# ArielleRosinski/pyGAT

Hardware: AMD Instinct MI355X
Metric: GAT-layer fwd+bwd edges/sec (higher is better)
Workload: dtype f32

## Files before the change

include/pygat_amd.h:

```cpp
#ifndef PYGAT_AMD_H
#define PYGAT_AMD_H

#include <stdint.h>
#include <stddef.h>

#ifdef __cplusplus
extern "C" {
#endif

#define PYGAT_ABI_VERSION 15

enum {
  PYGAT_OK = 0,
  PYGAT_EINVAL = -1,
  PYGAT_EHIP = -2,
  PYGAT_ENODEV = -3
};

enum {
  PYGAT_F_ELU = 1,
  PYGAT_F_SKIP = 2,
  PYGAT_F_MAIN_ONLY = 4,
  PYGAT_F_FIXUP_ONLY = 8
};

// ... 63 lines not shown
typedef struct {
  int n;
  int64_t nnz;
  const int32_t* rowptr;
  const int32_t* edge_rc;
  int slot_edges;
  const int32_t* slot_begin;
  const int32_t* cut_rows;
  int n_cut;
  int n_cut_wide;
  int64_t slot_first;
  int64_t slot_count;
  const int32_t* slot_meta;
  const int32_t* slot_order;
  const int32_t* user_row;
} pygat_graph;

int pygat_edge_pairs(int n, const int32_t* rowptr, const int32_t* col, int32_t* edge_rc, void* stream);

int pygat_slot_bounds(int n, int64_t nnz, const int32_t* rowptr, const int32_t* edge_rc, int slot_edges,
                      int32_t* slot_begin, void* stream);
int pygat_slot_meta(int n, int64_t nnz, const int32_t* rowptr, const int32_t* edge_rc, int slot_edges,
                    const int32_t* slot_begin, int32_t* slot_meta, void* stream);

size_t pygat_partials_bytes(int64_t nnz, int slot_edges, int H, int Fp);

int pygat_head_group(int n, int H, int Fo);

int pygat_gat_forward_phases_ok(int n, int H, int Fo);
int pygat_gat_forward(const pygat_graph* g, int H, int Fo, float alpha, int flags,
                      const float* Wh, const float* s, const float* a_pad, const float* sk,
// ... 119 lines not shown
```

pygat_amd/_lib.py:

```python
from __future__ import annotations

import ctypes as C
import os

import torch

_HERE = os.path.dirname(os.path.abspath(__file__))
LIB_PATH = os.path.join(_HERE, "libpygat_amd.so")
from .config import config as _config
if _config.lib_path:
    LIB_PATH = os.path.abspath(_config.lib_path)

ABI_VERSION = 15
F_ELU = 1
F_SKIP = 2
F_MAIN_ONLY = 4
F_FIXUP_ONLY = 8

SYMBOLS = [
    "pygat_abi_version", "pygat_last_error", "pygat_padded_width", "pygat_device_count",
    "pygat_device_name", "pygat_kernel_footprint", "pygat_default_gemm_mode", "pygat_dense_row_counts", "pygat_scan_workspace_bytes",
    "pygat_exclusive_scan_i32", "pygat_dense_fill_cols", "pygat_csr_symmetric_perm",
    "pygat_gemm_workspace_bytes", "pygat_gemm_f32", "pygat_gemm_f32_blocked", "pygat_project_blocked", "pygat_wgrad_blocked", "pygat_pack_params", "pygat_pack_params_heads", "pygat_stack_heads", "pygat_stack_heads_padded", "pygat_project", "pygat_attn_scores",
    "pygat_unpack_wgrad",
    "pygat_edge_pairs", "pygat_slot_bounds", "pygat_slot_meta", "pygat_partials_bytes", "pygat_head_group", "pygat_gat_forward", "pygat_gat_forward_phases_ok", "pygat_gat_forward_tail", "pygat_gat_backward_col_tail", "pygat_gat_backward_tail", "pygat_project_tail_blocked", "pygat_head_mean",
    "pygat_gat_backward_prepare", "pygat_gat_backward_row", "pygat_gat_backward_col", "pygat_gat_backward_rowsum",
    "pygat_gat_backward_col_da_bytes", "pygat_a_grad_fold",
    "pygat_agrad_workspace_bytes", "pygat_a_grad", "pygat_wgrad_workspace_bytes", "pygat_wgrad",
# ... 13 lines not shown


class OutSegments(C.Structure):
    _fields_ = [("nseg", C.c_int), ("col_start", C.c_int32 * (MAX_SEGMENTS + 1)), ("ptr", C.c_void_p * MAX_SEGMENTS),
                ("ld", C.c_int64 * MAX_SEGMENTS)]


class ColBlocks(C.Structure):
    _fields_ = [("w", C.c_int), ("stride", C.c_int64)]


class Graph(C.Structure):
    _fields_ = [("n", C.c_int), ("nnz", C.c_int64), ("rowptr", C.c_void_p), ("edge_rc", C.c_void_p),
                ("slot_edges", C.c_int), ("slot_begin", C.c_void_p), ("cut_rows", C.c_void_p),
                ("n_cut", C.c_int), ("n_cut_wide", C.c_int), ("slot_first", C.c_int64), ("slot_count", C.c_int64),
                ("slot_meta", C.c_void_p), ("slot_order", C.c_void_p), ("user_row", C.c_void_p)]


def _load():
    if not os.path.exists(LIB_PATH):
        raise ImportError(
            f"pygat_amd: {LIB_PATH} not found. Build it with `python -c 'import __graft_entry__ as g; "
            f"g.build()'` or `make -C pygat_amd/csrc`. There is no CPU/PyTorch fallback for the hot path.")
    lib = C.CDLL(LIB_PATH)
    missing = [s for s in SYMBOLS if not hasattr(lib, s)]
    if missing:
        raise ImportError(f"pygat_amd: {LIB_PATH} lacks symbols {missing}")
    p, i, i64, f, sz = C.c_void_p, C.c_int, C.c_int64, C.c_float, C.c_size_t
    lib.pygat_abi_version.restype = i
    lib.pygat_last_error.restype = C.c_char_p
    lib.pygat_padded_width.argtypes = [i]
# ... 113 lines not shown
```

pygat_amd/config.py:

```python
from __future__ import annotations

import os
from dataclasses import dataclass, fields
from typing import Optional


def _flag(name: str, default: bool) -> bool:
    v = os.environ.get(name)
    return default if v is None else v not in ("0", "", "false", "False")


def _opt_flag(name: str) -> Optional[bool]:
    v = os.environ.get(name)
    return None if v is None else v == "1"


def _opt_int(name: str) -> Optional[int]:
    v = os.environ.get(name)
    return int(v) if v else None


@dataclass(frozen=True)
class Config:
    lib_path: Optional[str]
    dist_chunks: int
    dropout_wide: bool
    sparse_max_density: float
    sparse_x: bool
    slot_edges: Optional[int]
    slot_meta: bool
    two_gather_backward: Optional[bool]
    backward: Optional[str]
    da_in_k4: bool
    k1_split_min_k: int
    overlap_backward: bool
    pad_k: bool
    renumber: bool
    tail: bool
    tail_fused: bool

    @staticmethod
    def from_env() -> "Config":
        return Config(
            lib_path=os.environ.get("PYGAT_AMD_LIB") or None,
            dist_chunks=int(os.environ.get("PYGAT_DIST_CHUNKS", 4)),
            dropout_wide=_flag("PYGAT_DROPOUT_WIDE", False),
            sparse_max_density=float(os.environ.get("PYGAT_SPARSE_MAX_DENSITY", 0.15)),
            sparse_x=_flag("PYGAT_SPARSE_X", True),
            slot_edges=_opt_int("PYGAT_SLOT_EDGES"),
            slot_meta=not _flag("PYGAT_NO_SLOT_META", False),
            two_gather_backward=_opt_flag("PYGAT_TWO_GATHER_BACKWARD"),
            backward=os.environ.get("PYGAT_BACKWARD") or None,
            da_in_k4=_flag("PYGAT_DA_IN_K4", True),
            k1_split_min_k=int(os.environ.get("PYGAT_K1_SPLIT_MIN_K", 128)),
            overlap_backward=_flag("PYGAT_OVERLAP_BACKWARD", False),
            pad_k=_flag("PYGAT_PAD_K", True),
            renumber=_flag("PYGAT_RENUMBER", True),
            tail=_flag("PYGAT_TAIL", True),
            tail_fused=_flag("PYGAT_TAIL_FUSED", True),
        )

    def describe(self) -> dict:
        return {f.name: getattr(self, f.name) for f in fields(self)}


config = Config.from_env()
```

pygat_amd/csrc/attn_common.h:

```cpp
#pragma once
#include "common.h"

namespace pygat {

constexpr int FIX_LIST_WAVES = 16;
__host__ __device__ constexpr int fix_rows_per_wave(int lpr) { return 64 / lpr >= 8 ? 4 : (64 / lpr >= 2 ? 2 : 1); }
constexpr int FIX_WIDE = 32;
constexpr int FIX_SCREEN = 8;
constexpr float NEG_BIG = -1.0e30f;

struct RowShape {
  int H, Fo, Fp, R, NCH;
  int fp_shift;
  int lph;
  int Htot;
  int64_t ldr;
  int64_t ldh;
  int64_t ldo;
};

static inline bool make_row_shape(int H, int Fo, RowShape* rs) {
  int Fp = padded_width(Fo);
  if (H <= 0 || Fp == 0) return false;
  rs->H = H; rs->Fo = Fo; rs->Fp = Fp; rs->R = H * Fp; rs->NCH = rs->R / 4;
// ... 75 lines not shown
  } while (0)

struct GraphDev {
  int n;
  int64_t nnz;
  const int32_t* rowptr;
  const int2* rc;
  int ts;
  const int32_t* sb;
  const int4* meta;
  const int32_t* cut;
  int n_cut, n_cut_wide;
  int64_t k0, kn;
  const int32_t* order;
  const int32_t* urow;
};

static inline int check_graph(const pygat_graph* g, GraphDev* d, int allow_slot_range = 0) {
  if (!g || !g->rowptr || !g->edge_rc || g->n <= 0 || g->nnz <= 0) {
    set_error("graph: null or empty (n=%d nnz=%lld)", g ? g->n : -1, g ? (long long)g->nnz : -1LL);
    return PYGAT_EINVAL;
  }
  if (g->nnz >= (int64_t)1 << 31) {
    set_error("graph: nnz %lld exceeds int32 edge indexing", (long long)g->nnz);
    return PYGAT_EINVAL;
  }
  if (g->slot_edges < 4 || (g->slot_edges & 3)) {
    set_error("graph: slot_edges=%d must be a multiple of 4, >= 4", g->slot_edges);
    return PYGAT_EINVAL;
  }
  d->n = g->n; d->nnz = g->nnz; d->rowptr = g->rowptr; d->rc = reinterpret_cast<const int2*>(g->edge_rc);
  d->ts = g->slot_edges; d->sb = g->slot_begin; d->meta = reinterpret_cast<const int4*>(g->slot_meta);
  if (g->slot_meta && !aligned16(g->slot_meta)) {
    set_error("graph: slot_meta must be 16-byte aligned");
    return PYGAT_EINVAL;
  }
  d->cut = g->cut_rows; d->n_cut = g->cut_rows ? g->n_cut : 0; d->n_cut_wide = g->cut_rows ? g->n_cut_wide : 0;
  if (d->n_cut < 0 || d->n_cut_wide < 0 || d->n_cut_wide > d->n_cut) {
    set_error("graph: bad cut-row list (n_cut=%d n_cut_wide=%d)", g->n_cut, g->n_cut_wide);
    return PYGAT_EINVAL;
  }
  const int64_t total = (g->nnz + g->slot_edges - 1) / g->slot_edges;
  d->k0 = 0; d->kn = total;
  d->order = g->slot_order;
  d->urow = g->user_row;
  if (g->slot_order && g->slot_count != 0) {
    set_error("graph: slot_order needs the whole slot range (slot_count = 0)");
    return PYGAT_EINVAL;
  }
  if (g->slot_count != 0) {
    if (!allow_slot_range || g->slot_first < 0 || g->slot_count < 0 || g->slot_first + g->slot_count > total ||
        (allow_slot_range == 2 && g->slot_first != 0)) {
      set_error("graph: slot range [%lld, +%lld) of %lld %s", (long long)g->slot_first, (long long)g->slot_count,
                (long long)total, allow_slot_range ? "is out of bounds (or not a prefix, for the column pass)"
                                                   : "is not supported by this entry point");
      return PYGAT_EINVAL;
    }
    d->k0 = g->slot_first; d->kn = g->slot_count;
  }
  return PYGAT_OK;
// ... 78 lines not shown
template <int LPR, int SPAN = 64>
__device__ __forceinline__ float slot_sum(float x) {
#pragma unroll
  for (int off = LPR; off < SPAN; off <<= 1) x += __shfl_xor(x, off);
  return x;
}
template <int LPR, int SPAN = 64>
__device__ __forceinline__ float4 slot_sum4(float4 v) {
#pragma unroll
  for (int off = LPR; off < SPAN; off <<= 1) {
    v.x += __shfl_xor(v.x, off); v.y += __shfl_xor(v.y, off);
    v.z += __shfl_xor(v.z, off); v.w += __shfl_xor(v.w, off);
  }
  return v;
}
#endif

}
```

pygat_amd/csrc/k2_forward.hip:

```cpp
#include "attn_common.h"

namespace pygat {

struct FwdArgs {
  GraphDev g;
  RowShape rs;
  float alpha;
  int flags;
  const float* Wh;
  int64_t ldwh;
  const float* s;
  const float* a_pad;
  const float* sk;
  const float* mask;
  float* out;
  float* hattn;
  float* m;
  float* Z;
  float* part;
  float* aneg;
  float* qneg;
};

__device__ __forceinline__ float lrelu(float z, float alpha) { return z > 0.f ? z : alpha * z; }
// ... 91 lines not shown
        float* o = a.out + io * ldo + (int64_t)h * Fo + f0;
        if (f0 + 0 < Fo) o[0] = pre.x;
        if (f0 + 1 < Fo) o[1] = pre.y;
        if (f0 + 2 < Fo) o[2] = pre.z;
        if (f0 + 3 < Fo) o[3] = pre.w;
      }
    }
    if (a.m && ((co >> 2) & (a.rs.lph - 1)) == 0) {
      a.m[(int64_t)i * ldh + h] = st.m[v];
      a.Z[(int64_t)i * ldh + h] = st.z[v];
      if constexpr (AUX) a.qneg[(int64_t)i * ldh + h] = mixed[v] ? st.zn[v] * rz : 0.f;
    }
  }
}

template <int VEC, bool AUX>
__device__ __forceinline__ void part_store(const FwdArgs& a, const LaneCols<VEC>& lc, float* p, const RowState<VEC, AUX>& st) {
  const int R = a.rs.R, H = a.rs.H;
#pragma unroll
  for (int v = 0; v < VEC; ++v) {
    if (!lc.valid[v]) continue;
    st4(p + lc.cofs[v], st.acc[v]);
    if constexpr (AUX) st4(p + R + 2 * H + lc.cofs[v], st.accn[v]);
    if (((lc.cofs[v] >> 2) & (a.rs.lph - 1)) == 0) {
      p[R + lc.head[v]] = st.m[v];
      p[R + H + lc.head[v]] = st.z[v];
      if constexpr (AUX) p[2 * R + 2 * H + lc.head[v]] = st.zn[v];
    }
  }
}
template <int VEC, bool AUX>
struct PartRec {
  float m[VEC], z[VEC];
  float4 acc[VEC];
  float zn[AUX ? VEC : 1];
  float4 accn[AUX ? VEC : 1];
};
template <int VEC, bool AUX>
__device__ __forceinline__ void part_load(const FwdArgs& a, const LaneCols<VEC>& lc, const float* p, PartRec<VEC, AUX>& r) {
  const int R = a.rs.R, H = a.rs.H;
#pragma unroll
  for (int v = 0; v < VEC; ++v) {
// ... 1 lines not shown
    if constexpr (AUX) { r.zn[v] = p[2 * R + 2 * H + lc.head[v]]; r.accn[v] = ld4(p + R + 2 * H + lc.cofs[v]); }
  }
}
template <int VEC, bool AUX>
__device__ __forceinline__ void part_merge(RowState<VEC, AUX>& st, const PartRec<VEC, AUX>& r) {
#pragma unroll
  for (int v = 0; v < VEC; ++v)
    merge_state<AUX>(st.m[v], st.z[v], st.acc[v], st.zn[AUX ? v : 0], st.accn[AUX ? v : 0], r.m[v], r.z[v], r.acc[v],
                     r.zn[AUX ? v : 0], r.accn[AUX ? v : 0]);
}

template <int LPR, int VEC, bool AUX, int LPH = 0, int CR = 0>
__device__ __forceinline__ void fwd_flush(const FwdArgs& a, const LaneCols<VEC>& lc, int64_t k, int i,
                                          bool is_head, bool is_tail, const RowState<VEC, AUX>& st) {
  if (is_head || is_tail) {
    part_store<VEC, AUX>(a, lc, a.part + (2 * k + (is_head ? 0 : 1)) * part_stride<AUX>(a.rs), st);
  } else {
    fwd_finish<LPR, VEC, AUX, LPH, CR>(a, lc, i, st);
  }
}

#ifndef PYGAT_K2_PREFETCH_ALL
#define PYGAT_K2_PREFETCH_ALL 0
#endif
#ifndef PYGAT_K2_PREFETCH_TRAIN
#define PYGAT_K2_PREFETCH_TRAIN 1
#endif
#ifndef PYGAT_K2_HEADLINE_WAVES
#define PYGAT_K2_HEADLINE_WAVES 4
#endif
#ifndef PYGAT_K2_DEEP
#define PYGAT_K2_DEEP 0
#endif
#ifndef PYGAT_K2_NARROW_U
#define PYGAT_K2_NARROW_U 4
#endif
template <int LPR, int VEC, bool V2, bool AUX, bool FAST, int LPH = 0, int CR = 0>
__global__ __launch_bounds__(256) __attribute__((amdgpu_waves_per_eu((AUX && FAST && VEC == 1 && LPR > 8) ? PYGAT_K2_HEADLINE_WAVES : 1))) void gat_fwd_kernel(FwdArgs a) {
  constexpr int EPW = 64 / LPR;
  constexpr bool NARROW = (VEC == 1 && LPR <= 8);
  constexpr bool PREF = NARROW || (PYGAT_K2_PREFETCH_ALL && VEC == 1) || (PYGAT_K2_PREFETCH_TRAIN && AUX && FAST && VEC == 1);
  constexpr int U = (VEC == 1) ? (NARROW ? PYGAT_K2_NARROW_U : 4) : 2;
  const int lane = threadIdx.x & 63;
  const int64_t kl = ((int64_t)blockIdx.x * (blockDim.x >> 6) + (threadIdx.x >> 6)) * EPW + lane / LPR;
  if (kl >= a.g.kn) return;
  const int64_t k = a.g.order ? a.g.order[kl] : a.g.k0 + kl;
  int64_t e0, e1;
  const int2* __restrict__ rc = a.g.rc;
  int r_first;
  bool head_partial, tail_known = false, tail_flag = false;
  if (a.g.meta) {
    const int4 mt = a.g.meta[k];
    e0 = mt.x; e1 = mt.y; r_first = mt.z;
    head_partial = (mt.w & 1) != 0; tail_known = true; tail_flag = (mt.w & 2) != 0;
  } else {
    slot_range(a.g, k, &e0, &e1);
    r_first = rc[e0].x;
    head_partial = a.g.rowptr[r_first] < e0;
  }
  const LaneCols<VEC> lc = lane_cols<LPR, VEC>(a.rs);
  const int R = CR ? CR : a.rs.R;
// ... 117 lines not shown
          st.reset();
        }
#pragma unroll
        for (int v = 0; v < VEC; ++v) {
          const float zz = sv[u][v] + tv[u][v];
          fold_edge<AUX>(st.m[v], st.z[v], st.acc[v], st.zn[AUX ? v : 0], st.accn[AUX ? v : 0],
                         V2 ? tv[u][v] : lrelu(zz, a.alpha), !(zz > 0.f), wv[u][v], mk[u][v]);
        }
      }
    }
  }
  const bool tail_partial = tail_known ? tail_flag : a.g.rowptr[cur + 1] > e1;
  fwd_flush<LPR, VEC, AUX, LPH, CR>(a, lc, k, cur, cur == r_first && head_partial, tail_partial, st);
}

template <int LPR, int VEC, bool AUX, int NW, int G = 64 / LPR>
__device__ __forceinline__ void fwd_merge_row(const FwdArgs& a, const LaneCols<VEC>& lc, float* fix_sm, int64_t k, int r,
                                              int npieces, bool wide, int w) {
  constexpr int PF = (VEC == 1) ? 4 : 2;
  const int lane = threadIdx.x & 63, slot = lane / LPR, g = slot % G;
  const int64_t PS = part_stride<AUX>(a.rs);
  RowState<VEC, AUX> st;
  st.reset();
  if (wide || w == 0) {
    const int nw = wide ? NW : 1;
    for (int q = (wide ? w : 0) * G * PF + g; q < npieces; q += nw * G * PF) {
      PartRec<VEC, AUX> rec[PF];
#pragma unroll
      for (int f = 0; f < PF; ++f) {
        const int qq = q + f * G;
        const int qc = qq < npieces ? qq : q;
        part_load<VEC, AUX>(a, lc, a.part + (qc == 0 ? 2 * k + 1 : 2 * (k + qc)) * PS, rec[f]);
      }
#pragma unroll
      for (int f = 0; f < PF; ++f)
        if (q + f * G < npieces) part_merge<VEC, AUX>(st, rec[f]);
    }
#pragma unroll
    for (int off = LPR; off < LPR * G; off <<= 1) {
#pragma unroll
      for (int v = 0; v < VEC; ++v) {
        const float mo = __shfl_xor(st.m[v], off), zo = __shfl_xor(st.z[v], off);
        float4 ao, no = make_float4(0.f, 0.f, 0.f, 0.f);
        float zno = 0.f;
        ao.x = __shfl_xor(st.acc[v].x, off); ao.y = __shfl_xor(st.acc[v].y, off);
        ao.z = __shfl_xor(st.acc[v].z, off); ao.w = __shfl_xor(st.acc[v].w, off);
        if constexpr (AUX) {
          zno = __shfl_xor(st.zn[v], off);
          no.x = __shfl_xor(st.accn[v].x, off); no.y = __shfl_xor(st.accn[v].y, off);
          no.z = __shfl_xor(st.accn[v].z, off); no.w = __shfl_xor(st.accn[v].w, off);
        }
        merge_state<AUX>(st.m[v], st.z[v], st.acc[v], st.zn[AUX ? v : 0], st.accn[AUX ? v : 0], mo, zo, ao, zno, no);
      }
    }
  }
  if (wide) {
    if (slot == 0) part_store<VEC, AUX>(a, lc, fix_sm + w * PS, st);
    __syncthreads();
    if (w == 0 && slot == 0) {
#pragma unroll
      for (int ww = 1; ww < NW; ++ww) {
        PartRec<VEC, AUX> rec;
        part_load<VEC, AUX>(a, lc, fix_sm + ww * PS, rec);
        part_merge<VEC, AUX>(st, rec);
      }
    }
    __syncthreads();
  }
  if (w == 0 && g == 0 && npieces > 0) fwd_finish<LPR, VEC, AUX>(a, lc, r, st);
}

template <int LPR, int VEC, bool AUX>
__global__ __launch_bounds__(256) void gat_fwd_fixup_kernel(FwdArgs a) {
  constexpr int EPW = 64 / LPR;
  constexpr int PF = (VEC == 1) ? 4 : 2;
  extern __shared__ __attribute__((aligned(16))) float fix_sm[];
  const int lane = threadIdx.x & 63, w = threadIdx.x >> 6;
  const int64_t kbase = a.g.k0 + (int64_t)blockIdx.x * FIX_SCREEN;
  const int64_t nslots = a.g.k0 + a.g.kn;
  int my_r = 0, my_end = 0;
  bool owner = false;
  if (lane < FIX_SCREEN && kbase + lane < nslots) {
    int64_t e0, e1;
    slot_range(a.g, kbase + lane, &e0, &e1);
// ... 77 lines not shown
extern "C" size_t pygat_partials_bytes(int64_t nnz, int slot_edges, int H, int Fp) {
  if (nnz <= 0 || slot_edges <= 0) return 0;
  const int64_t nslots = (nnz + slot_edges - 1) / slot_edges;
  return (size_t)(2 * nslots) * (size_t)(2 * H * Fp + 3 * H) * sizeof(float);
}

static int launch_forward(const pygat_graph* g, int H, int Fo, float alpha, int flags, const float* Wh, int v2,
                          const float* s, const float* a_pad, const float* sk, const float* att_mask, float* out,
                          float* hattn, float* m, float* Z, float* aneg, float* qneg, void* part, void* stream) {
  FwdArgs a;
  int rc = check_graph(g, &a.g, v2 ? 2 : 1);
  if (rc) return rc;
  const int Fp = padded_width(Fo);
  PYGAT_REQUIRE(H > 0 && Fp > 0, "gat_forward: unsupported H=%d F'=%d", H, Fo);
  PYGAT_REQUIRE(Wh && (s || v2) && a_pad && part, "gat_forward: null Wh/s/a_pad/part");
  PYGAT_REQUIRE(out || hattn, "gat_forward: need out and/or hattn");
  PYGAT_REQUIRE(!(flags & PYGAT_F_SKIP) || sk, "gat_forward: PYGAT_F_SKIP without sk");
  PYGAT_REQUIRE((m == nullptr) == (Z == nullptr), "gat_forward: m and Z must be given together");
  PYGAT_REQUIRE((aneg == nullptr) == (qneg == nullptr) && (!aneg || (m && !v2 && aligned16(aneg))),
                "gat_forward: aneg and qneg come together, need m/Z, 16-byte alignment and the v1 layer");
  PYGAT_REQUIRE(aligned16(Wh) && aligned16(part) && aligned16(a_pad) && (!sk || aligned16(sk)) && (!hattn || aligned16(hattn)) &&
                    (!out || Fo != Fp || aligned16(out)),
                "gat_forward: row tables must be 16-byte aligned");
  hipStream_t st = (hipStream_t)stream;
  const int64_t nslots = a.g.kn;
  const int hg = v2 ? H : head_group_fwd_n(a.g.n, H, Fp);
  const bool do_main = !(flags & PYGAT_F_FIXUP_ONLY), do_fix = !(flags & PYGAT_F_MAIN_ONLY);
  PYGAT_REQUIRE(do_main || do_fix, "gat_forward: PYGAT_F_MAIN_ONLY and PYGAT_F_FIXUP_ONLY exclude each other");
  PYGAT_REQUIRE((do_main && do_fix) || hg >= H, "gat_forward: a single phase needs the level in one head window (pygat_gat_forward_phases_ok)");
  flags &= ~(PYGAT_F_MAIN_ONLY | PYGAT_F_FIXUP_ONLY);
// ... 24 lines not shown
    if (!do_main) {}
    else if (v2) PYGAT_FWD(true, false, false);
    else if (aux && fast && lpr == 32 && vec == 1 && a.rs.lph == 4)
      if (a.rs.R == 128 && a.rs.ldr == 128 && a.rs.ldh == 8 && a.rs.ldo == 128 && a.rs.Fo == 16 && a.ldwh == 128 && !(flags & PYGAT_F_SKIP))
        hipLaunchKernelGGL((gat_fwd_kernel<32, 1, false, true, true, 4, 128>), dim3(blocks), dim3(bt), 0, st, a);
      else
        hipLaunchKernelGGL((gat_fwd_kernel<32, 1, false, true, true, 4>), dim3(blocks), dim3(bt), 0, st, a);
    else if (aux && fast) PYGAT_FWD(false, true, true);
    else if (aux) PYGAT_FWD(false, true, false);
    else PYGAT_FWD(false, false, false);
#undef PYGAT_FWD
    PYGAT_CHECK_LAUNCH("gat_forward");
    const bool listed = a.g.cut != nullptr;
    const int fix_waves = listed ? FIX_LIST_WAVES : 4;
    const size_t fix_lds = fix_waves * (size_t)(aux ? part_stride<true>(a.rs) : part_stride<false>(a.rs)) * sizeof(float);
    const unsigned fb = listed ? (unsigned)(a.g.n_cut_wide + cdiv(a.g.n_cut - a.g.n_cut_wide, FIX_LIST_WAVES * fix_rows_per_wave(lpr)))
                               : (unsigned)cdiv(nslots, FIX_SCREEN);
    if ((listed && a.g.n_cut == 0) || !do_fix) continue;
#define PYGAT_FIX(AUXV)                                                                                               \
    do {                                                                                                              \
      if (listed) {                                                                                                   \
        PYGAT_DISPATCH_LANES(lpr, vec, hipLaunchKernelGGL((gat_fwd_fixup_list_kernel<LPR, VEC, AUXV>), dim3(fb),     \
                                                          dim3(64 * FIX_LIST_WAVES), fix_lds, st, a));                \
      } else {                                                                                                        \
        PYGAT_DISPATCH_LANES(lpr, vec, hipLaunchKernelGGL((gat_fwd_fixup_kernel<LPR, VEC, AUXV>), dim3(fb), dim3(256), \
                                                          fix_lds, st, a));                                           \
      }                                                                                                               \
    } while (0)
    if (aux) PYGAT_FIX(true); else PYGAT_FIX(false);
#undef PYGAT_FIX
    PYGAT_CHECK_LAUNCH("gat_forward_fixup");
  }
  return PYGAT_OK;
// ... 55 lines not shown
```

pygat_amd/graph.py:

```python
from __future__ import annotations

import ctypes as C
import weakref
from typing import Optional, Tuple

import torch

from . import _lib
from ._lib import lib, check
from .config import config as _config

SLOT_ORDER_FN = None
FORCED_SLOT_EDGES = _config.slot_edges
USE_SLOT_META = _config.slot_meta

DEFAULT_SLOT_EDGES = 64


def auto_slot_edges(nnz: int) -> int:
    if FORCED_SLOT_EDGES:
        return int(FORCED_SLOT_EDGES)
    ts = DEFAULT_SLOT_EDGES
    while ts > 4 and nnz // ts < 8192:
        ts //= 2
    return ts


def slot_edges_for(row_floats: int, base: int = DEFAULT_SLOT_EDGES) -> int:
    return min(base, 32) if row_floats <= 16 else base
# ... 7 lines not shown
    return None if t is None else t.data_ptr()


class _Pattern:

    def __init__(self, rowptr: torch.Tensor, col: torch.Tensor, slot_edges: int, user_row: Optional[torch.Tensor] = None):
        self.rowptr, self.col, self.slot_edges = rowptr, col, slot_edges
        self.user_row = user_row
        self.n = rowptr.numel() - 1
        self.nnz = col.numel()
        self.edge_rc = torch.empty(self.nnz, 2, dtype=torch.int32, device=rowptr.device)
        with torch.cuda.device(rowptr.device):
            check(lib.pygat_edge_pairs(self.n, rowptr.data_ptr(), col.data_ptr(), self.edge_rc.data_ptr(), _stream()),
                  "edge_pairs")
        self._alt = {}
        self.struct = self._make(slot_edges, True)

    def _make(self, slot_edges: int, snapped: bool):
        key = (slot_edges, snapped)
        if key not in self._alt:
            sb = None
            if snapped:
                nslots = -(-self.nnz // slot_edges)
                sb = torch.empty(nslots + 1, dtype=torch.int32, device=self.rowptr.device)
                with torch.cuda.device(self.rowptr.device):
                    check(lib.pygat_slot_bounds(self.n, self.nnz, self.rowptr.data_ptr(), self.edge_rc.data_ptr(),
                                                slot_edges, sb.data_ptr(), _stream()), "slot_bounds")
            cut, n_cut, n_wide = None, 0, 0
            if snapped:
                sbl = sb.long()
# ... 8 lines not shown
                    order = torch.argsort(pieces, descending=True, stable=True)
                    cut = torch.stack([k, r_last[k], pieces], 1)[order].to(torch.int32).contiguous()
                    n_cut, n_wide = int(k.numel()), int((pieces > 32).sum().item())
                else:
                    cut = torch.zeros(1, 3, dtype=torch.int32, device=self.rowptr.device)
            meta = torch.empty(-(-self.nnz // slot_edges), 4, dtype=torch.int32, device=self.rowptr.device)
            with torch.cuda.device(self.rowptr.device):
                check(lib.pygat_slot_meta(self.n, self.nnz, self.rowptr.data_ptr(), self.edge_rc.data_ptr(), slot_edges, _ptr(sb),
                                          meta.data_ptr(), _stream()), "slot_meta")
            if not USE_SLOT_META:
                meta = None
            order = SLOT_ORDER_FN(self, meta) if (SLOT_ORDER_FN is not None and meta is not None) else None
            st = _lib.Graph(self.n, self.nnz, _ptr(self.rowptr), _ptr(self.edge_rc), slot_edges, _ptr(sb), _ptr(cut),
                            n_cut, n_wide, 0, 0, _ptr(meta), _ptr(order), _ptr(self.user_row))
            self._alt[key] = (st, sb, cut, meta, order)
        return self._alt[key][0]

    def row_chunks(self, nchunks: int, slot_edges: Optional[int] = None, nslots: Optional[int] = None, row_end: Optional[int] = None):
        ts = slot_edges or self.slot_edges
        key = ("chunks", ts, nchunks, nslots)
        if key not in self._alt:
            base = self._make(ts, True)
            _, sb, cut, meta, _order = self._alt[(ts, True)]
            all_slots = sb.numel() - 1
            nslots = all_slots if nslots is None else int(nslots)
            sbl, rp = sb.long(), self.rowptr.long()
            first_row = self.edge_rc[sbl[:-1], 0].long()
            starts_row = rp[first_row] == sbl[:-1]
            ok = torch.nonzero(starts_row[:nslots]).flatten()
            borders = [0]
            for c in range(1, nchunks):
# ... 7 lines not shown
                r0 = int(first_row[b0])
                r1 = int(first_row[b1]) if b1 < nslots else (self.n if (row_end is None or nslots == all_slots) else int(row_end))
                sub, n_cut, n_wide = None, 0, 0
                if cut is not None:
                    sel = (cut[:, 0] >= b0) & (cut[:, 0] < b1)
                    sub = cut[sel].contiguous()
                    n_cut, n_wide = int(sub.shape[0]), int((sub[:, 2] > 32).sum().item()) if sub.numel() else 0
                    if n_cut == 0:
                        sub = cut[:1].contiguous()
                st = _lib.Graph(self.n, self.nnz, _ptr(self.rowptr), _ptr(self.edge_rc), ts, _ptr(sb), _ptr(sub), n_cut,
                                n_wide, b0, b1 - b0, _ptr(meta), None, _ptr(self.user_row))
                out.append((st, r0, r1))
                keep.append(sub)
            self._alt[key] = (out, keep)
            del base
        return [(C.byref(st), r0, r1) for st, r0, r1 in self._alt[key][0]]

    def self_loop_tail(self, slot_edges: Optional[int] = None):
        ts = slot_edges or self.slot_edges
        key = ("tail", ts)
        if key not in self._alt:
            st = self._make(ts, True)
            _, sb, cut, meta, order = self._alt[(ts, True)]
            out = None
            if meta is not None and order is None:
                rp = self.rowptr.long()
                deg = rp[1:] - rp[:-1]
                n1 = int((deg > 1).sum().item())
                if n1 < self.n and bool((deg[n1:] == 1).all().item()) and bool((self.col[rp[n1]:].long() == torch.arange(n1, self.n, device=self.col.device)).all().item()):
                    first_row = meta[:, 2].long()
                    k = int(torch.searchsorted(first_row, torch.tensor(n1, device=first_row.device)).item())
                    if 0 < k < meta.shape[0]:
                        row_first = int(first_row[k].item())
                        pre = _lib.Graph()
                        C.memmove(C.byref(pre), C.byref(st), C.sizeof(_lib.Graph))
                        pre.slot_first, pre.slot_count = 0, k
                        out = (row_first, k, pre)
            self._alt[key] = out
        t = self._alt[key]
        return None if t is None else (t[0], t[1], C.byref(t[2]))

    def ref(self, slot_edges: Optional[int] = None, snapped: bool = True):
        return C.byref(self._make(slot_edges or self.slot_edges, snapped))


class _UnmappedPattern:

    def __init__(self, base: "_Pattern"):
        self._base = base
        self._copies = {}
        self.user_row = None

    def __getattr__(self, name):
        return getattr(self._base, name)

    def _strip(self, key, struct_ref):
        if key not in self._copies:
            st = _lib.Graph()
            C.memmove(C.byref(st), struct_ref, C.sizeof(_lib.Graph))
            st.user_row = None
            self._copies[key] = st
        return C.byref(self._copies[key])

    def ref(self, slot_edges: Optional[int] = None, snapped: bool = True):
        return self._strip(("ref", slot_edges or self._base.slot_edges, snapped), self._base.ref(slot_edges, snapped))

    def row_chunks(self, nchunks: int, slot_edges: Optional[int] = None, nslots: Optional[int] = None, row_end: Optional[int] = None):
        out = self._base.row_chunks(nchunks, slot_edges, nslots, row_end)
        return [(self._strip(("chunk", slot_edges or self._base.slot_edges, nchunks, nslots, c), ref), r0, r1)
                for c, (ref, r0, r1) in enumerate(out)]

    def self_loop_tail(self, slot_edges: Optional[int] = None):
        t = self._base.self_loop_tail(slot_edges)
        return None if t is None else (t[0], t[1], self._strip(("tail", slot_edges or self._base.slot_edges), t[2]))


class InternalOrderView:
    degree_sorted = True
    user_row = None
    _ordered = None

    def __init__(self, g_int: "CSRGraph", to_user: torch.Tensor, to_internal: torch.Tensor):
        self.base = g_int
        self.n, self.nnz, self.device, self.slot_edges, self.symmetric = g_int.n, g_int.nnz, g_int.device, g_int.slot_edges, g_int.symmetric
        self.fwd = _UnmappedPattern(g_int.fwd)
        self.bwd = self.fwd if g_int.bwd is g_int.fwd else _UnmappedPattern(g_int.bwd)
        self.perm_t, self.perm_f = g_int.perm_t, g_int.perm_f
        self.to_user, self.to_internal = to_user, to_internal

# ... 173 lines not shown
```

Baseline: 4.134 billion.

## Merge cut-row partials inside the forward kernel via arrival counters

Adds per-cut-row atomic arrival counters so the last slot to finish a row split across slots merges the partial softmax states inline, inside the forward kernel. Only narrow cut rows (up to 32 pieces) are handled this way; wide rows keep the separate fix-up launch. Partial stores use agent-scope atomic write-through so other workgroups see them before merging. This is meant to remove most of the fix-up kernel launch and its extra pass over the partials, at the cost of atomics, fences and possible divergence in the main kernel.

```diff
diff --git a/include/pygat_amd.h b/include/pygat_amd.h
--- a/include/pygat_amd.h
+++ b/include/pygat_amd.h
@@ -8,7 +8,7 @@
 extern "C" {
 #endif
 
-#define PYGAT_ABI_VERSION 15
+#define PYGAT_ABI_VERSION 16
 
 enum {
   PYGAT_OK = 0,
@@ -102,7 +102,12 @@
   const int32_t* slot_meta;
   const int32_t* slot_order;
   const int32_t* user_row;
+  const int32_t* slot_cut;
+  const int32_t* cut_all;
+  uint32_t* merge_cnt;
+  int n_cut_all;
 } pygat_graph;
+enum { PYGAT_MERGE_FWD = 0, PYGAT_MERGE_FWD_V2 = 1, PYGAT_MERGE_COL = 2, PYGAT_MERGE_PASSES = 3 };
 
 int pygat_edge_pairs(int n, const int32_t* rowptr, const int32_t* col, int32_t* edge_rc, void* stream);
 
diff --git a/pygat_amd/_lib.py b/pygat_amd/_lib.py
--- a/pygat_amd/_lib.py
+++ b/pygat_amd/_lib.py
@@ -11,7 +11,7 @@
 if _config.lib_path:
     LIB_PATH = os.path.abspath(_config.lib_path)
 
-ABI_VERSION = 15
+ABI_VERSION = 16
 F_ELU = 1
 F_SKIP = 2
 F_MAIN_ONLY = 4
@@ -55,7 +55,9 @@
     _fields_ = [("n", C.c_int), ("nnz", C.c_int64), ("rowptr", C.c_void_p), ("edge_rc", C.c_void_p),
                 ("slot_edges", C.c_int), ("slot_begin", C.c_void_p), ("cut_rows", C.c_void_p),
                 ("n_cut", C.c_int), ("n_cut_wide", C.c_int), ("slot_first", C.c_int64), ("slot_count", C.c_int64),
-                ("slot_meta", C.c_void_p), ("slot_order", C.c_void_p), ("user_row", C.c_void_p)]
+                ("slot_meta", C.c_void_p), ("slot_order", C.c_void_p), ("user_row", C.c_void_p),
+                ("slot_cut", C.c_void_p), ("cut_all", C.c_void_p), ("merge_cnt", C.c_void_p), ("n_cut_all", C.c_int)]
+MERGE_PASSES = 3
 
 
 def _load():
diff --git a/pygat_amd/config.py b/pygat_amd/config.py
--- a/pygat_amd/config.py
+++ b/pygat_amd/config.py
@@ -38,6 +38,7 @@
     renumber: bool
     tail: bool
     tail_fused: bool
+    inkernel_merge: bool
 
     @staticmethod
     def from_env() -> "Config":
@@ -58,6 +59,7 @@
             renumber=_flag("PYGAT_RENUMBER", True),
             tail=_flag("PYGAT_TAIL", True),
             tail_fused=_flag("PYGAT_TAIL_FUSED", True),
+            inkernel_merge=_flag("PYGAT_INKERNEL_MERGE", True),
         )
 
     def describe(self) -> dict:
diff --git a/pygat_amd/csrc/attn_common.h b/pygat_amd/csrc/attn_common.h
--- a/pygat_amd/csrc/attn_common.h
+++ b/pygat_amd/csrc/attn_common.h
@@ -113,6 +113,10 @@
   int64_t k0, kn;
   const int32_t* order;
   const int32_t* urow;
+  const int2* slot_cut;
+  const int32_t* cut_all;
+  uint32_t* merge_cnt;
+  int n_cut_all;
 };
 
 static inline int check_graph(const pygat_graph* g, GraphDev* d, int allow_slot_range = 0) {
@@ -143,6 +147,18 @@
   d->k0 = 0; d->kn = total;
   d->order = g->slot_order;
   d->urow = g->user_row;
+  d->slot_cut = reinterpret_cast<const int2*>(g->slot_cut); d->cut_all = g->cut_all; d->merge_cnt = g->merge_cnt;
+  d->n_cut_all = g->slot_cut ? g->n_cut_all : 0;
+  if (g->slot_cut && (!g->cut_all || !g->merge_cnt || g->n_cut_all < 0 || ((uintptr_t)g->slot_cut & 7))) {
+    set_error("graph: slot_cut needs cut_all, merge_cnt, n_cut_all >= 0 and 8-byte alignment");
+    return PYGAT_EINVAL;
+  }
+  d->slot_cut = reinterpret_cast<const int2*>(g->slot_cut); d->cut_all = g->cut_all; d->merge_cnt = g->merge_cnt;
+  d->n_cut_all = g->slot_cut ? g->n_cut_all : 0;
+  if (g->slot_cut && (!g->cut_all || !g->merge_cnt || g->n_cut_all < 0 || ((uintptr_t)g->slot_cut & 7))) {
+    set_error("graph: slot_cut needs cut_all, merge_cnt, n_cut_all >= 0 and 8-byte alignment");
+    return PYGAT_EINVAL;
+  }
   if (g->slot_order && g->slot_count != 0) {
     set_error("graph: slot_order needs the whole slot range (slot_count = 0)");
     return PYGAT_EINVAL;
@@ -251,6 +267,64 @@
   }
   return v;
 }
+
+__device__ __forceinline__ void st4_wt(float* p, float4 v) {
+  unsigned long long* q = reinterpret_cast<unsigned long long*>(p);
+  __hip_atomic_store(q, (unsigned long long)__float_as_uint(v.x) | ((unsigned long long)__float_as_uint(v.y) << 32),
+                     __ATOMIC_RELAXED, __HIP_MEMORY_SCOPE_AGENT);
+  __hip_atomic_store(q + 1, (unsigned long long)__float_as_uint(v.z) | ((unsigned long long)__float_as_uint(v.w) << 32),
+                     __ATOMIC_RELAXED, __HIP_MEMORY_SCOPE_AGENT);
+}
+__device__ __forceinline__ void st1_wt(float* p, float v) { __hip_atomic_store(p, v, __ATOMIC_RELAXED, __HIP_MEMORY_SCOPE_AGENT); }
+__device__ __forceinline__ void merge_drain() { asm volatile("s_waitcnt vmcnt(0)" ::: "memory"); }
+__device__ __forceinline__ bool merge_arrive(const GraphDev& g, int pass, int c) {
+  uint32_t* cnt = g.merge_cnt + (int64_t)pass * g.n_cut_all + c;
+  const uint32_t pieces = (uint32_t)g.cut_all[3 * c + 2];
+  const uint32_t old = __hip_atomic_fetch_add(cnt, 1u, __ATOMIC_RELAXED, __HIP_MEMORY_SCOPE_AGENT);
+  if (old + 1u != pieces) return false;
+  __hip_atomic_store(cnt, 0u, __ATOMIC_RELAXED, __HIP_MEMORY_SCOPE_AGENT);
+  return true;
+}
+__device__ __forceinline__ void merge_acquire() {
+  __builtin_amdgcn_fence(__ATOMIC_ACQUIRE, "agent");
+  asm volatile("s_waitcnt vmcnt(0)" ::: "memory");
+}
+struct MergeJobs {
+  unsigned long long mh, mt;
+  int jh, jt;
+};
+template <int LPR>
+__device__ __forceinline__ bool merge_arrivals(const GraphDev& g, int pass, int2 sc, MergeJobs& j) {
+  const bool lead = ((threadIdx.x & 63) & (LPR - 1)) == 0;
+  merge_drain();
+  j.jh = (lead && sc.x >= 0 && merge_arrive(g, pass, sc.x)) ? sc.x : -1;
+  j.jt = (lead && sc.y >= 0 && merge_arrive(g, pass, sc.y)) ? sc.y : -1;
+  j.mh = __ballot(j.jh >= 0);
+  j.mt = __ballot(j.jt >= 0);
+  if ((j.mh | j.mt) == 0ull) return false;
+  merge_acquire();
+  return true;
+}
+__device__ __forceinline__ int merge_next(MergeJobs& j) {
+  if (j.mh) { const int src = __ffsll((long long)j.mh) - 1; j.mh &= j.mh - 1; return __shfl(j.jh, src); }
+  if (j.mt) { const int src = __ffsll((long long)j.mt) - 1; j.mt &= j.mt - 1; return __shfl(j.jt, src); }
+  return -1;
+}
+template <int LPR, typename BATCH>
+__device__ __forceinline__ void merge_jobs(MergeJobs& j, BATCH&& batch) {
+  constexpr int RPW = fix_rows_per_wave(LPR), G = 64 / LPR / RPW;
+  const int row = ((threadIdx.x & 63) / LPR) / G;
+  for (;;) {
+    int b[RPW];
+#pragma unroll
+    for (int r = 0; r < RPW; ++r) b[r] = merge_next(j);
+    if (b[0] < 0) break;
+    int mine = -1;
+#pragma unroll
+    for (int r = 0; r < RPW; ++r) mine = (r == row) ? b[r] : mine;
+    batch(mine);
+  }
+}
 #endif
 
 }
diff --git a/pygat_amd/csrc/k2_forward.hip b/pygat_amd/csrc/k2_forward.hip
--- a/pygat_amd/csrc/k2_forward.hip
+++ b/pygat_amd/csrc/k2_forward.hip
@@ -129,18 +129,20 @@
   }
 }
 
-template <int VEC, bool AUX>
+template <int VEC, bool AUX, bool WT = false>
 __device__ __forceinline__ void part_store(const FwdArgs& a, const LaneCols<VEC>& lc, float* p, const RowState<VEC, AUX>& st) {
   const int R = a.rs.R, H = a.rs.H;
+  auto s4 = [](float* q, float4 x) { if constexpr (WT) st4_wt(q, x); else st4(q, x); };
+  auto s1 = [](float* q, float x) { if constexpr (WT) st1_wt(q, x); else *q = x; };
 #pragma unroll
   for (int v = 0; v < VEC; ++v) {
     if (!lc.valid[v]) continue;
-    st4(p + lc.cofs[v], st.acc[v]);
-    if constexpr (AUX) st4(p + R + 2 * H + lc.cofs[v], st.accn[v]);
+    s4(p + lc.cofs[v], st.acc[v]);
+    if constexpr (AUX) s4(p + R + 2 * H + lc.cofs[v], st.accn[v]);
     if (((lc.cofs[v] >> 2) & (a.rs.lph - 1)) == 0) {
-      p[R + lc.head[v]] = st.m[v];
-      p[R + H + lc.head[v]] = st.z[v];
-      if constexpr (AUX) p[2 * R + 2 * H + lc.head[v]] = st.zn[v];
+      s1(p + R + lc.head[v], st.m[v]);
+      s1(p + R + H + lc.head[v], st.z[v]);
+      if constexpr (AUX) s1(p + 2 * R + 2 * H + lc.head[v], st.zn[v]);
     }
   }
 }
@@ -172,7 +174,9 @@
 __device__ __forceinline__ void fwd_flush(const FwdArgs& a, const LaneCols<VEC>& lc, int64_t k, int i,
                                           bool is_head, bool is_tail, const RowState<VEC, AUX>& st) {
   if (is_head || is_tail) {
-    part_store<VEC, AUX>(a, lc, a.part + (2 * k + (is_head ? 0 : 1)) * part_stride<AUX>(a.rs), st);
+    float* p = a.part + (2 * k + (is_head ? 0 : 1)) * part_stride<AUX>(a.rs);
+    if (a.g.slot_cut) part_store<VEC, AUX, true>(a, lc, p, st);
+    else part_store<VEC, AUX>(a, lc, p, st);
   } else {
     fwd_finish<LPR, VEC, AUX, LPH, CR>(a, lc, i, st);
   }
@@ -193,16 +197,14 @@
 #ifndef PYGAT_K2_NARROW_U
 #define PYGAT_K2_NARROW_U 4
 #endif
-template <int LPR, int VEC, bool V2, bool AUX, bool FAST, int LPH = 0, int CR = 0>
-__global__ __launch_bounds__(256) __attribute__((amdgpu_waves_per_eu((AUX && FAST && VEC == 1 && LPR > 8) ? PYGAT_K2_HEADLINE_WAVES : 1))) void gat_fwd_kernel(FwdArgs a) {
-  constexpr int EPW = 64 / LPR;
+template <int LPR, int VEC, bool AUX>
+__device__ __forceinline__ void fwd_merge_inline(const FwdArgs& a, int pass, int2 sc);
+
+template <int LPR, int VEC, bool V2, bool AUX, bool FAST, int LPH, int CR>
+__device__ __forceinline__ void fwd_walk(const FwdArgs& a, const int64_t k) {
   constexpr bool NARROW = (VEC == 1 && LPR <= 8);
   constexpr bool PREF = NARROW || (PYGAT_K2_PREFETCH_ALL && VEC == 1) || (PYGAT_K2_PREFETCH_TRAIN && AUX && FAST && VEC == 1);
   constexpr int U = (VEC == 1) ? (NARROW ? PYGAT_K2_NARROW_U : 4) : 2;
-  const int lane = threadIdx.x & 63;
-  const int64_t kl = ((int64_t)blockIdx.x * (blockDim.x >> 6) + (threadIdx.x >> 6)) * EPW + lane / LPR;
-  if (kl >= a.g.kn) return;
-  const int64_t k = a.g.order ? a.g.order[kl] : a.g.k0 + kl;
   int64_t e0, e1;
   const int2* __restrict__ rc = a.g.rc;
   int r_first;
@@ -350,46 +352,66 @@
   fwd_flush<LPR, VEC, AUX, LPH, CR>(a, lc, k, cur, cur == r_first && head_partial, tail_partial, st);
 }
 
+template <int LPR, int VEC, bool V2, bool AUX, bool FAST, int LPH = 0, int CR = 0>
+__global__ __launch_bounds__(256) __attribute__((amdgpu_waves_per_eu((AUX && FAST && VEC == 1 && LPR > 8) ? PYGAT_K2_HEADLINE_WAVES : 1))) void gat_fwd_kernel(FwdArgs a) {
+  constexpr int EPW = 64 / LPR;
+  const int lane = threadIdx.x & 63;
+  const int64_t kl = ((int64_t)blockIdx.x * (blockDim.x >> 6) + (threadIdx.x >> 6)) * EPW + lane / LPR;
+  int2 sc = make_int2(-1, -1);
+  if (kl < a.g.kn) {
+    const int64_t k = a.g.order ? a.g.order[kl] : a.g.k0 + kl;
+    if (a.g.slot_cut) sc = a.g.slot_cut[k];
+    fwd_walk<LPR, VEC, V2, AUX, FAST, LPH, CR>(a, k);
+  }
+  if (a.g.slot_cut && __ballot(sc.x >= 0 || sc.y >= 0)) fwd_merge_inline<LPR, VEC, AUX>(a, V2 ? PYGAT_MERGE_FWD_V2 : PYGAT_MERGE_FWD, sc);
+}
+
+template <int LPR, int VEC, bool AUX, int G>
+__device__ __forceinline__ void fwd_merge_wave(const FwdArgs& a, const LaneCols<VEC>& lc, int64_t k, int npieces, int w, int nw,
+                                               RowState<VEC, AUX>& st) {
+  constexpr int PF = (VEC == 1) ? 4 : 2;
+  const int g = ((threadIdx.x & 63) / LPR) % G;
+  const int64_t PS = part_stride<AUX>(a.rs);
+  st.reset();
+  for (int q = w * G * PF + g; q < npieces; q += nw * G * PF) {
+    PartRec<VEC, AUX> rec[PF];
+#pragma unroll
+    for (int f = 0; f < PF; ++f) {
+      const int qq = q + f * G;
+      const int qc = qq < npieces ? qq : q;
+      part_load<VEC, AUX>(a, lc, a.part + (qc == 0 ? 2 * k + 1 : 2 * (k + qc)) * PS, rec[f]);
+    }
+#pragma unroll
+    for (int f = 0; f < PF; ++f)
+      if (q + f * G < npieces) part_merge<VEC, AUX>(st, rec[f]);
+  }
+#pragma unroll
+  for (int off = LPR; off < LPR * G; off <<= 1) {
+#pragma unroll
+    for (int v = 0; v < VEC; ++v) {
+      const float mo = __shfl_xor(st.m[v], off), zo = __shfl_xor(st.z[v], off);
+      float4 ao, no = make_float4(0.f, 0.f, 0.f, 0.f);
+      float zno = 0.f;
+      ao.x = __shfl_xor(st.acc[v].x, off); ao.y = __shfl_xor(st.acc[v].y, off);
+      ao.z = __shfl_xor(st.acc[v].z, off); ao.w = __shfl_xor(st.acc[v].w, off);
+      if constexpr (AUX) {
+        zno = __shfl_xor(st.zn[v], off);
+        no.x = __shfl_xor(st.accn[v].x, off); no.y = __shfl_xor(st.accn[v].y, off);
+        no.z = __shfl_xor(st.accn[v].z, off); no.w = __shfl_xor(st.accn[v].w, off);
+      }
+      merge_state<AUX>(st.m[v], st.z[v], st.acc[v], st.zn[AUX ? v : 0], st.accn[AUX ? v : 0], mo, zo, ao, zno, no);
+    }
+  }
+}
+
 template <int LPR, int VEC, bool AUX, int NW, int G = 64 / LPR>
 __device__ __forceinline__ void fwd_merge_row(const FwdArgs& a, const LaneCols<VEC>& lc, float* fix_sm, int64_t k, int r,
                                               int npieces, bool wide, int w) {
-  constexpr int PF = (VEC == 1) ? 4 : 2;
   const int lane = threadIdx.x & 63, slot = lane / LPR, g = slot % G;
   const int64_t PS = part_stride<AUX>(a.rs);
   RowState<VEC, AUX> st;
   st.reset();
-  if (wide || w == 0) {
-    const int nw = wide ? NW : 1;
-    for (int q = (wide ? w : 0) * G * PF + g; q < npieces; q += nw * G * PF) {
-      PartRec<VEC, AUX> rec[PF];
-#pragma unroll
-      for (int f = 0; f < PF; ++f) {
-        const int qq = q + f * G;
-        const int qc = qq < npieces ? qq : q;
-        part_load<VEC, AUX>(a, lc, a.part + (qc == 0 ? 2 * k + 1 : 2 * (k + qc)) * PS, rec[f]);
-      }
-#pragma unroll
-      for (int f = 0; f < PF; ++f)
-        if (q + f * G < npieces) part_merge<VEC, AUX>(st, rec[f]);
-    }
-#pragma unroll
-    for (int off = LPR; off < LPR * G; off <<= 1) {
-#pragma unroll
-      for (int v = 0; v < VEC; ++v) {
-        const float mo = __shfl_xor(st.m[v], off), zo = __shfl_xor(st.z[v], off);
-        float4 ao, no = make_float4(0.f, 0.f, 0.f, 0.f);
-        float zno = 0.f;
-        ao.x = __shfl_xor(st.acc[v].x, off); ao.y = __shfl_xor(st.acc[v].y, off);
-        ao.z = __shfl_xor(st.acc[v].z, off); ao.w = __shfl_xor(st.acc[v].w, off);
-        if constexpr (AUX) {
-          zno = __shfl_xor(st.zn[v], off);
-          no.x = __shfl_xor(st.accn[v].x, off); no.y = __shfl_xor(st.accn[v].y, off);
-          no.z = __shfl_xor(st.accn[v].z, off); no.w = __shfl_xor(st.accn[v].w, off);
-        }
-        merge_state<AUX>(st.m[v], st.z[v], st.acc[v], st.zn[AUX ? v : 0], st.accn[AUX ? v : 0], mo, zo, ao, zno, no);
-      }
-    }
-  }
+  if (wide || w == 0) fwd_merge_wave<LPR, VEC, AUX, G>(a, lc, k, npieces, wide ? w : 0, wide ? NW : 1, st);
   if (wide) {
     if (slot == 0) part_store<VEC, AUX>(a, lc, fix_sm + w * PS, st);
     __syncthreads();
@@ -404,6 +426,19 @@
     __syncthreads();
   }
   if (w == 0 && g == 0 && npieces > 0) fwd_finish<LPR, VEC, AUX>(a, lc, r, st);
+}
+
+template <int LPR, int VEC, bool AUX>
+__device__ __forceinline__ void fwd_merge_inline(const FwdArgs& a, int pass, int2 sc) {
+  MergeJobs j;
+  if (!merge_arrivals<LPR>(a.g, pass, sc, j)) return;
+  const LaneCols<VEC> lc = lane_cols<LPR, VEC>(a.rs);
+  constexpr int RPW = fix_rows_per_wave(LPR), G = 64 / LPR / RPW;
+  merge_jobs<LPR>(j, [&](int mine) {
+    const int c = mine >= 0 ? mine : 0;
+    fwd_merge_row<LPR, VEC, AUX, FIX_LIST_WAVES, G>(a, lc, nullptr, a.g.cut_all[3 * c], a.g.cut_all[3 * c + 1],
+                                                    mine >= 0 ? a.g.cut_all[3 * c + 2] : 0, false, 0);
+  });
 }
 
 template <int LPR, int VEC, bool AUX>
@@ -511,6 +546,7 @@
   const int Fp = padded_width(Fo);
   PYGAT_REQUIRE(H > 0 && Fp > 0, "gat_forward: unsupported H=%d F'=%d", H, Fo);
   PYGAT_REQUIRE(Wh && (s || v2) && a_pad && part, "gat_forward: null Wh/s/a_pad/part");
+  PYGAT_REQUIRE(!a.g.slot_cut || a.g.cut, "gat_forward: slot_cut needs the cut-row list (its wide rows keep their fix-up launch)");
   PYGAT_REQUIRE(out || hattn, "gat_forward: need out and/or hattn");
   PYGAT_REQUIRE(!(flags & PYGAT_F_SKIP) || sk, "gat_forward: PYGAT_F_SKIP without sk");
   PYGAT_REQUIRE((m == nullptr) == (Z == nullptr), "gat_forward: m and Z must be given together");
@@ -565,9 +601,10 @@
     const bool listed = a.g.cut != nullptr;
     const int fix_waves = listed ? FIX_LIST_WAVES : 4;
     const size_t fix_lds = fix_waves * (size_t)(aux ? part_stride<true>(a.rs) : part_stride<false>(a.rs)) * sizeof(float);
-    const unsigned fb = listed ? (unsigned)(a.g.n_cut_wide + cdiv(a.g.n_cut - a.g.n_cut_wide, FIX_LIST_WAVES * fix_rows_per_wave(lpr)))
+    const unsigned fb = a.g.slot_cut ? (unsigned)a.g.n_cut_wide
+                      : listed ? (unsigned)(a.g.n_cut_wide + cdiv(a.g.n_cut - a.g.n_cut_wide, FIX_LIST_WAVES * fix_rows_per_wave(lpr)))
                                : (unsigned)cdiv(nslots, FIX_SCREEN);
-    if ((listed && a.g.n_cut == 0) || !do_fix) continue;
+    if ((listed && a.g.n_cut == 0) || !do_fix || fb == 0) continue;
 #define PYGAT_FIX(AUXV)                                                                                               \
     do {                                                                                                              \
       if (listed) {                                                                                                   \
diff --git a/pygat_amd/graph.py b/pygat_amd/graph.py
--- a/pygat_amd/graph.py
+++ b/pygat_amd/graph.py
@@ -13,6 +13,8 @@
 SLOT_ORDER_FN = None
 FORCED_SLOT_EDGES = _config.slot_edges
 USE_SLOT_META = _config.slot_meta
+INKERNEL_MERGE = _config.inkernel_merge
+FIX_WIDE = 32
 
 DEFAULT_SLOT_EDGES = 64
 
@@ -50,6 +52,7 @@
             check(lib.pygat_edge_pairs(self.n, rowptr.data_ptr(), col.data_ptr(), self.edge_rc.data_ptr(), _stream()),
                   "edge_pairs")
         self._alt = {}
+        self._merge = {}
         self.struct = self._make(slot_edges, True)
 
     def _make(self, slot_edges: int, snapped: bool):
@@ -88,7 +91,38 @@
             st = _lib.Graph(self.n, self.nnz, _ptr(self.rowptr), _ptr(self.edge_rc), slot_edges, _ptr(sb), _ptr(cut),
                             n_cut, n_wide, 0, 0, _ptr(meta), _ptr(order), _ptr(self.user_row))
             self._alt[key] = (st, sb, cut, meta, order)
+            if snapped:
+                self._merge[slot_edges] = self._merge_tables(-(-self.nnz // slot_edges), cut, n_cut)
         return self._alt[key][0]
+
+    @staticmethod
+    def _merge_tables(nslots: int, cut: torch.Tensor, n_cut: int):
+        dev = cut.device
+        sc = torch.full((nslots, 2), -1, dtype=torch.int32, device=dev)
+        if n_cut:
+            c = cut[:n_cut].long()
+            ids = torch.arange(n_cut, device=dev)
+            keep = c[:, 2] <= FIX_WIDE
+            k, p, ids = c[keep, 0], c[keep, 2], ids[keep]
+            sc[k, 1] = ids.to(torch.int32)
+            rep = p - 1
+            first = torch.repeat_interleave(torch.cumsum(rep, 0) - rep, rep)
+            j = torch.arange(int(rep.sum().item()), device=dev) - first + 1
+            sc[torch.repeat_interleave(k, rep) + j, 0] = torch.repeat_interleave(ids, rep).to(torch.int32)
+        cnt = torch.zeros(_lib.MERGE_PASSES * n_cut + 1, dtype=torch.int32, device=dev)
+        return sc, cnt, cut, n_cut
+
+    def _merged(self, key, st, slot_edges: int):
+        if not INKERNEL_MERGE or slot_edges not in self._merge:
+            return st
+        key = ("merged",) + tuple(key)
+        if key not in self._alt:
+            sc, cnt, cut, n_cut = self._merge[slot_edges]
+            cp = _lib.Graph()
+            C.memmove(C.byref(cp), C.byref(st), C.sizeof(_lib.Graph))
+            cp.slot_cut, cp.cut_all, cp.merge_cnt, cp.n_cut_all = sc.data_ptr(), cut.data_ptr(), cnt.data_ptr(), n_cut
+            self._alt[key] = cp
+        return self._alt[key]
 
     def row_chunks(self, nchunks: int, slot_edges: Optional[int] = None, nslots: Optional[int] = None, row_end: Optional[int] = None):
         ts = slot_edges or self.slot_edges
@@ -126,7 +160,7 @@
                 keep.append(sub)
             self._alt[key] = (out, keep)
             del base
-        return [(C.byref(st), r0, r1) for st, r0, r1 in self._alt[key][0]]
+        return [(C.byref(self._merged(key + (c,), st, ts)), r0, r1) for c, (st, r0, r1) in enumerate(self._alt[key][0])]
 
     def self_loop_tail(self, slot_edges: Optional[int] = None):
         ts = slot_edges or self.slot_edges
@@ -150,10 +184,12 @@
                         out = (row_first, k, pre)
             self._alt[key] = out
         t = self._alt[key]
-        return None if t is None else (t[0], t[1], C.byref(t[2]))
+        return None if t is None else (t[0], t[1], C.byref(self._merged(key, t[2], ts)))
 
     def ref(self, slot_edges: Optional[int] = None, snapped: bool = True):
-        return C.byref(self._make(slot_edges or self.slot_edges, snapped))
+        ts = slot_edges or self.slot_edges
+        st = self._make(ts, snapped)
+        return C.byref(self._merged(("ref", ts), st, ts) if snapped else st)
 
 
 class _UnmappedPattern:
@@ -175,16 +211,16 @@
         return C.byref(self._copies[key])
 
     def ref(self, slot_edges: Optional[int] = None, snapped: bool = True):
-        return self._strip(("ref", slot_edges or self._base.slot_edges, snapped), self._base.ref(slot_edges, snapped))
+        return self._strip(("ref", slot_edges or self._base.slot_edges, snapped, INKERNEL_MERGE), self._base.ref(slot_edges, snapped))
 
     def row_chunks(self, nchunks: int, slot_edges: Optional[int] = None, nslots: Optional[int] = None, row_end: Optional[int] = None):
         out = self._base.row_chunks(nchunks, slot_edges, nslots, row_end)
-        return [(self._strip(("chunk", slot_edges or self._base.slot_edges, nchunks, nslots, c), ref), r0, r1)
+        return [(self._strip(("chunk", slot_edges or self._base.slot_edges, nchunks, nslots, c, INKERNEL_MERGE), ref), r0, r1)
                 for c, (ref, r0, r1) in enumerate(out)]
 
     def self_loop_tail(self, slot_edges: Optional[int] = None):
         t = self._base.self_loop_tail(slot_edges)
-        return None if t is None else (t[0], t[1], self._strip(("tail", slot_edges or self._base.slot_edges), t[2]))
+        return None if t is None else (t[0], t[1], self._strip(("tail", slot_edges or self._base.slot_edges, INKERNEL_MERGE), t[2]))
 
 
 class InternalOrderView:
```

Result: slower. 3.959 billion (median of 2 runs) (-4.2%).
